# POSTECH-CVLab/PyTorch-StudioGAN

Hardware: AMD Instinct MI355X
Metric: images/sec (G+D step) BigGAN ImageNet-128 bs256 (higher is better)
Workload: dtype bf16

## Files before the change

pytorch-studiogan_amd/csrc/attn.hip:

```cpp
#include "common.h"
#include "lds_tile.h"
#include "../../include/sgamd.h"

#ifndef AT_UNROLL
#define AT_UNROLL 1
#endif
#ifndef AT_WAVES
#define AT_WAVES(NCG) ((NCG) <= 2 ? 3 : 2)
#endif

__device__ __forceinline__ u32x4 at_gfrag(const bf16_t* base, long long row, int ld, int c, int C) {
  u32x4 z = {0u, 0u, 0u, 0u};
  return (c < C) ? *(const u32x4*)(base + row * ld + c) : z;
}

#ifndef AT_THR
#define AT_THR 8.0f
#endif
template <int NCG>
__global__ __launch_bounds__(256) __attribute__((amdgpu_waves_per_eu(AT_WAVES(NCG), AT_WAVES(NCG)))) void k_attn_fwd_flash(const bf16_t* theta, const bf16_t* phi, const bf16_t* g, float* lse, bf16_t* O, float* O32,
                                                        int HW, int HW4, int Dp, int Cg) {
  constexpr int KC = 256;
  constexpr float LOG2E = 1.4426950408889634f;
  extern __shared__ __attribute__((aligned(16))) char at_smem[];
  char* kimg = at_smem;
  char* vimg = at_smem + KC * 64;
  const int tid = threadIdx.x, lane = tid & 63, wave = __builtin_amdgcn_readfirstlane(tid >> 6);
  const int b = blockIdx.y;
  const int q = blockIdx.x * 128 + wave * 32 + (lane & 31);
  const int h = lane >> 5;
  const long long qrow = (long long)b * HW + q;
  const bf16x8_t qf0 = __builtin_bit_cast(bf16x8_t, at_gfrag(theta, qrow, Dp, 8 * h, Dp));
  const bf16x8_t qf1 = __builtin_bit_cast(bf16x8_t, at_gfrag(theta, qrow, Dp, 16 + 8 * h, Dp));
  float m = -3.0e38f;
  float m2 = m * LOG2E;
  float l = 0.f;
  f32x16 o[NCG];
#pragma unroll
  for (int cg = 0; cg < NCG; cg++)
#pragma unroll
    for (int r = 0; r < 16; r++) o[cg][r] = 0.f;
  for (int k0 = 0; k0 < HW4; k0 += KC) {
    __syncthreads();
    lt_stage_cols<4>(kimg, phi + ((long long)b * HW4 + k0) * Dp, KC, Dp, 0, Dp, wave, lane);
#pragma unroll
    for (int cg = 0; cg < NCG; cg++) lt_stage_cols<4>(vimg + cg * KC * 64, g + ((long long)b * HW4 + k0) * Cg, KC, Cg, cg * 32, Cg, wave, lane);
    __syncthreads();
#pragma unroll AT_UNROLL
    for (int kc = 0; kc < KC / 32; kc++) {
      f32x16 s;
#pragma unroll
      for (int r = 0; r < 16; r++) s[r] = 0.f;
      s = __builtin_amdgcn_mfma_f32_32x32x16_bf16(lt_frag(kimg, kc, 0, lane), qf0, s, 0, 0, 0);
      s = __builtin_amdgcn_mfma_f32_32x32x16_bf16(lt_frag(kimg, kc, 1, lane), qf1, s, 0, 0, 0);
      float bm = s[0];
#pragma unroll
      for (int r = 1; r < 16; r++) bm = fmaxf(bm, s[r]);
      bm = lt_half_max(bm);
      if (bm > m + AT_THR) {
        const float alpha = __builtin_amdgcn_exp2f((m - bm) * LOG2E);
        l *= alpha;
#pragma unroll
        for (int cg = 0; cg < NCG; cg++)
#pragma unroll
          for (int r = 0; r < 16; r++) o[cg][r] *= alpha;
        m = bm;
        m2 = m * LOG2E;
      }
      float p[16];
#pragma unroll
      for (int r = 0; r < 16; r++) { p[r] = __builtin_amdgcn_exp2f(__builtin_fmaf(s[r], LOG2E, -m2)); l += p[r]; }
      u32x4 pa, pb;
#pragma unroll
      for (int i = 0; i < 4; i++) { pa[i] = pack2bf(p[2 * i], p[2 * i + 1]); pb[i] = pack2bf(p[8 + 2 * i], p[8 + 2 * i + 1]); }
      const bf16x8_t pfa = __builtin_bit_cast(bf16x8_t, pa), pfb = __builtin_bit_cast(bf16x8_t, pb);
#pragma unroll
      for (int cg = 0; cg < NCG; cg++) {
        const char* vi = vimg + cg * KC * 64;
        o[cg] = __builtin_amdgcn_mfma_f32_32x32x16_bf16(lt_vfrag(vi, kc * 32 + 4 * h, lane), pfa, o[cg], 0, 0, 0);
        o[cg] = __builtin_amdgcn_mfma_f32_32x32x16_bf16(lt_vfrag(vi, kc * 32 + 16 + 4 * h, lane), pfb, o[cg], 0, 0, 0);
      }
    }
  }
  l = lt_half_sum(l);
  const float inv = 1.f / l;
  if (h == 0) lse[qrow] = m + __logf(l);
  bf16_t* orow = O + qrow * Cg;
#pragma unroll
  for (int cg = 0; cg < NCG; cg++)
#pragma unroll
    for (int g4 = 0; g4 < 4; g4++) {
      const int c0 = cg * 32 + 8 * g4 + 4 * h;
      if (c0 < Cg) {
        const f32x4 f = {o[cg][4 * g4 + 0] * inv, o[cg][4 * g4 + 1] * inv, o[cg][4 * g4 + 2] * inv, o[cg][4 * g4 + 3] * inv};
        u32x2 v = {pack2bf(f[0], f[1]), pack2bf(f[2], f[3])};
        *(u32x2*)(orow + c0) = v;
        if (O32) *(f32x4*)(O32 + qrow * Cg + c0) = f;
      }
    }
}

template <int NCG> __global__ __launch_bounds__(256) __attribute__((amdgpu_waves_per_eu(AT_WAVES(NCG), AT_WAVES(NCG)))) void k_attn_bwd_q(const bf16_t* theta, const bf16_t* phi, const bf16_t* g, const bf16_t* dO, const float* Oin,
                                                                        const float* lse, float* delta_out, bf16_t* dtheta, int HW, int HW4, int Dp, int Cg) {
  constexpr int KC = 256;
  extern __shared__ __attribute__((aligned(16))) char at_smem[];
  char* kimg = at_smem;
  char* vimg = at_smem + KC * 64;
  const int tid = threadIdx.x, lane = tid & 63, wave = __builtin_amdgcn_readfirstlane(tid >> 6);
  const int b = blockIdx.y;
  const int q = blockIdx.x * 128 + wave * 32 + (lane & 31);
  const int h = lane >> 5;
  const long long qrow = (long long)b * HW + q;
  const bf16x8_t qf0 = __builtin_bit_cast(bf16x8_t, at_gfrag(theta, qrow, Dp, 8 * h, Dp));
  const bf16x8_t qf1 = __builtin_bit_cast(bf16x8_t, at_gfrag(theta, qrow, Dp, 16 + 8 * h, Dp));
  bf16x8_t df[NCG][2];
#pragma unroll
  for (int cg = 0; cg < NCG; cg++)
#pragma unroll
    for (int t = 0; t < 2; t++) df[cg][t] = __builtin_bit_cast(bf16x8_t, at_gfrag(dO, qrow, Cg, cg * 32 + 16 * t + 8 * h, Cg));
  float delta = 0.f;
  const float ls2 = lse[qrow] * 1.4426950408889634f;
  if (Oin) {
#pragma unroll
    for (int cg = 0; cg < NCG; cg++)
#pragma unroll
      for (int t = 0; t < 2; t++) {
        const int c0 = cg * 32 + 16 * t + 8 * h;
        if (c0 < Cg) {
          const f32x4 oa = *(const f32x4*)(Oin + qrow * Cg + c0), ob = *(const f32x4*)(Oin + qrow * Cg + c0 + 4);
          const u32x4 dv = __builtin_bit_cast(u32x4, df[cg][t]);
          delta += oa[0] * __uint_as_float(dv[0] << 16) + oa[1] * __uint_as_float(dv[0] & 0xffff0000u) + oa[2] * __uint_as_float(dv[1] << 16) + oa[3] * __uint_as_float(dv[1] & 0xffff0000u)
                 + ob[0] * __uint_as_float(dv[2] << 16) + ob[1] * __uint_as_float(dv[2] & 0xffff0000u) + ob[2] * __uint_as_float(dv[3] << 16) + ob[3] * __uint_as_float(dv[3] & 0xffff0000u);
        }
      }
    delta = lt_half_sum(delta);
  }
  f32x16 dth;
#pragma unroll
  for (int r = 0; r < 16; r++) dth[r] = 0.f;
  for (int pass = Oin ? 1 : 0; pass < 2; pass++) {
    for (int k0 = 0; k0 < HW4; k0 += KC) {
      __syncthreads();
      lt_stage_cols<4>(kimg, phi + ((long long)b * HW4 + k0) * Dp, KC, Dp, 0, Dp, wave, lane);
#pragma unroll
      for (int cg = 0; cg < NCG; cg++) lt_stage_cols<4>(vimg + cg * KC * 64, g + ((long long)b * HW4 + k0) * Cg, KC, Cg, cg * 32, Cg, wave, lane);
      __syncthreads();
#pragma unroll AT_UNROLL
      for (int kb = 0; kb < KC / 32; kb++) {
        f32x16 s, dp;
#pragma unroll
        for (int r = 0; r < 16; r++) { s[r] = 0.f; dp[r] = 0.f; }
        s = __builtin_amdgcn_mfma_f32_32x32x16_bf16(lt_frag(kimg, kb, 0, lane), qf0, s, 0, 0, 0);
        s = __builtin_amdgcn_mfma_f32_32x32x16_bf16(lt_frag(kimg, kb, 1, lane), qf1, s, 0, 0, 0);
#pragma unroll
        for (int cg = 0; cg < NCG; cg++)
#pragma unroll
          for (int t = 0; t < 2; t++)
            dp = __builtin_amdgcn_mfma_f32_32x32x16_bf16(lt_frag(vimg + cg * KC * 64, kb, t, lane), df[cg][t], dp, 0, 0, 0);
        if (pass == 0) {
#pragma unroll
          for (int r = 0; r < 16; r++) delta += __builtin_amdgcn_exp2f(__builtin_fmaf(s[r], 1.4426950408889634f, -ls2)) * dp[r];
        } else {
          float o[16];
#pragma unroll
          for (int r = 0; r < 16; r++) o[r] = __builtin_amdgcn_exp2f(__builtin_fmaf(s[r], 1.4426950408889634f, -ls2)) * (dp[r] - delta);
          u32x4 da, db;
#pragma unroll
          for (int i = 0; i < 4; i++) { da[i] = pack2bf(o[2 * i], o[2 * i + 1]); db[i] = pack2bf(o[8 + 2 * i], o[8 + 2 * i + 1]); }
          dth = __builtin_amdgcn_mfma_f32_32x32x16_bf16(lt_vfrag(kimg, kb * 32 + 4 * h, lane), __builtin_bit_cast(bf16x8_t, da), dth, 0, 0, 0);
          dth = __builtin_amdgcn_mfma_f32_32x32x16_bf16(lt_vfrag(kimg, kb * 32 + 16 + 4 * h, lane), __builtin_bit_cast(bf16x8_t, db), dth, 0, 0, 0);
        }
      }
    }
    if (pass == 0) delta = lt_half_sum(delta);
  }
  if (h == 0) delta_out[qrow] = delta;
  bf16_t* trow = dtheta + qrow * Dp;
#pragma unroll
  for (int g4 = 0; g4 < 4; g4++) {
    const int c0 = 8 * g4 + 4 * h;
    if (c0 < Dp) {
      u32x2 v = {pack2bf(dth[4 * g4 + 0], dth[4 * g4 + 1]), pack2bf(dth[4 * g4 + 2], dth[4 * g4 + 3])};
      *(u32x2*)(trow + c0) = v;
    }
  }
}

template <int NCG> __global__ __launch_bounds__(256) __attribute__((amdgpu_waves_per_eu(AT_WAVES(NCG), AT_WAVES(NCG)))) void k_attn_bwd_k(const bf16_t* theta, const bf16_t* phi, const bf16_t* g, const bf16_t* dO, const float* lse,
                                                                        const float* delta, bf16_t* dphi, bf16_t* dg, int HW, int HW4, int Dp, int Cg) {
  constexpr int QC = 256;
  extern __shared__ __attribute__((aligned(16))) char at_smem[];
  char* timg = at_smem;
  char* oimg = at_smem + QC * 64;
  float* st = (float*)(at_smem + (1 + NCG) * QC * 64);
  float* dl = st + QC;
  const int tid = threadIdx.x, lane = tid & 63, wave = __builtin_amdgcn_readfirstlane(tid >> 6);
  const int b = blockIdx.y;
  const int key = blockIdx.x * 128 + wave * 32 + (lane & 31);
  const int h = lane >> 5;
  const long long krow = (long long)b * HW4 + key;
  const bf16x8_t kf0 = __builtin_bit_cast(bf16x8_t, at_gfrag(phi, krow, Dp, 8 * h, Dp));
  const bf16x8_t kf1 = __builtin_bit_cast(bf16x8_t, at_gfrag(phi, krow, Dp, 16 + 8 * h, Dp));
  bf16x8_t gf[NCG][2];
#pragma unroll
  for (int cg = 0; cg < NCG; cg++)
#pragma unroll
    for (int t = 0; t < 2; t++) gf[cg][t] = __builtin_bit_cast(bf16x8_t, at_gfrag(g, krow, Cg, cg * 32 + 16 * t + 8 * h, Cg));
  f32x16 dph, dgt[NCG];
#pragma unroll
  for (int r = 0; r < 16; r++) dph[r] = 0.f;
#pragma unroll
  for (int cg = 0; cg < NCG; cg++)
#pragma unroll
    for (int r = 0; r < 16; r++) dgt[cg][r] = 0.f;
  for (int q0 = 0; q0 < HW; q0 += QC) {
    __syncthreads();
    lt_stage_cols<4>(timg, theta + ((long long)b * HW + q0) * Dp, QC, Dp, 0, Dp, wave, lane);
#pragma unroll
    for (int cg = 0; cg < NCG; cg++) lt_stage_cols<4>(oimg + cg * QC * 64, dO + ((long long)b * HW + q0) * Cg, QC, Cg, cg * 32, Cg, wave, lane);
    if (tid < QC) { st[tid] = lse[(long long)b * HW + q0 + tid] * 1.4426950408889634f; dl[tid] = delta[(long long)b * HW + q0 + tid]; }
    __syncthreads();
#pragma unroll AT_UNROLL
    for (int qb = 0; qb < QC / 32; qb++) {
      f32x16 s, dp;
#pragma unroll
      for (int r = 0; r < 16; r++) { s[r] = 0.f; dp[r] = 0.f; }
      s = __builtin_amdgcn_mfma_f32_32x32x16_bf16(lt_frag(timg, qb, 0, lane), kf0, s, 0, 0, 0);
      s = __builtin_amdgcn_mfma_f32_32x32x16_bf16(lt_frag(timg, qb, 1, lane), kf1, s, 0, 0, 0);
#pragma unroll
      for (int cg = 0; cg < NCG; cg++)
#pragma unroll
        for (int t = 0; t < 2; t++)
          dp = __builtin_amdgcn_mfma_f32_32x32x16_bf16(lt_frag(oimg + cg * QC * 64, qb, t, lane), gf[cg][t], dp, 0, 0, 0);
      float pr[16], ds[16];
#pragma unroll
      for (int r = 0; r < 16; r++) {
        const int qi = qb * 32 + (r & 3) + 8 * (r >> 2) + 4 * h;
        pr[r] = __builtin_amdgcn_exp2f(__builtin_fmaf(s[r], 1.4426950408889634f, -st[qi]));
        ds[r] = pr[r] * (dp[r] - dl[qi]);
      }
      u32x4 pa, pb, da, db;
#pragma unroll
      for (int i = 0; i < 4; i++) {
        pa[i] = pack2bf(pr[2 * i], pr[2 * i + 1]); pb[i] = pack2bf(pr[8 + 2 * i], pr[8 + 2 * i + 1]);
        da[i] = pack2bf(ds[2 * i], ds[2 * i + 1]); db[i] = pack2bf(ds[8 + 2 * i], ds[8 + 2 * i + 1]);
      }
#pragma unroll
      for (int cg = 0; cg < NCG; cg++) {
        const char* oi = oimg + cg * QC * 64;
        dgt[cg] = __builtin_amdgcn_mfma_f32_32x32x16_bf16(lt_vfrag(oi, qb * 32 + 4 * h, lane), __builtin_bit_cast(bf16x8_t, pa), dgt[cg], 0, 0, 0);
        dgt[cg] = __builtin_amdgcn_mfma_f32_32x32x16_bf16(lt_vfrag(oi, qb * 32 + 16 + 4 * h, lane), __builtin_bit_cast(bf16x8_t, pb), dgt[cg], 0, 0, 0);
      }
      dph = __builtin_amdgcn_mfma_f32_32x32x16_bf16(lt_vfrag(timg, qb * 32 + 4 * h, lane), __builtin_bit_cast(bf16x8_t, da), dph, 0, 0, 0);
      dph = __builtin_amdgcn_mfma_f32_32x32x16_bf16(lt_vfrag(timg, qb * 32 + 16 + 4 * h, lane), __builtin_bit_cast(bf16x8_t, db), dph, 0, 0, 0);
    }
  }
  bf16_t* prow = dphi + krow * Dp;
  bf16_t* grow = dg + krow * Cg;
#pragma unroll
  for (int g4 = 0; g4 < 4; g4++) {
    const int c0 = 8 * g4 + 4 * h;
    if (c0 < Dp) {
      u32x2 v = {pack2bf(dph[4 * g4 + 0], dph[4 * g4 + 1]), pack2bf(dph[4 * g4 + 2], dph[4 * g4 + 3])};
      *(u32x2*)(prow + c0) = v;
    }
  }
#pragma unroll
  for (int cg = 0; cg < NCG; cg++)
#pragma unroll
    for (int g4 = 0; g4 < 4; g4++) {
      const int c0 = cg * 32 + 8 * g4 + 4 * h;
      if (c0 < Cg) {
        u32x2 v = {pack2bf(dgt[cg][4 * g4 + 0], dgt[cg][4 * g4 + 1]), pack2bf(dgt[cg][4 * g4 + 2], dgt[cg][4 * g4 + 3])};
        *(u32x2*)(grow + c0) = v;
      }
    }
}

static bool at_ok(int B, int HW, int HW4, int Dp) {
  return B > 0 && B <= 65535 && HW % 128 == 0 && HW4 % 256 == 0 && Dp % 8 == 0 && Dp >= 8 && Dp <= 32;
}
extern "C" int sg_attn_fwd_flash_ok(int B, int HW, int HW4, int Dp, int Cg) {
  return (at_ok(B, HW, HW4, Dp) && Cg % 8 == 0 && Cg >= 8 && Cg <= 128) ? 1 : 0;
}
extern "C" int sg_attn_fwd_fused(const void* theta, const void* phi, const void* g, float* lse, void* O, float* O32, int B, int HW, int HW4, int Dp, int Cg, sg_stream_t s) {
  SG_CHECK(theta && phi && g && lse && O, "sg_attn_fwd_fused: null");
  SG_CHECK(sg_attn_fwd_flash_ok(B, HW, HW4, Dp, Cg) == 1, "sg_attn_fwd_fused: unsupported shape");
  const int ncg = (Cg + 31) / 32;
  SgProfScope prof((hipStream_t)s, (double)B * HW * ((Dp + Cg) * 2.0 + 4.0) + (double)B * HW4 * (Dp + Cg) * 2.0, 5);
  const dim3 grid(HW / 128, B), blk(256);
  hipStream_t st = (hipStream_t)s;
#define ATL_LAUNCH(N)                                                                                                                     \
  {                                                                                                                                        \
    static const bool ok = lt_allow_lds(k_attn_fwd_flash<N>, (1 + N) * 16384);                                                             \
    SG_CHECK(ok, "sg_attn_fwd_fused: LDS attribute");                                                                                      \
    hipLaunchKernelGGL((k_attn_fwd_flash<N>), grid, blk, (1 + N) * 16384, st, (const bf16_t*)theta, (const bf16_t*)phi, (const bf16_t*)g, lse, (bf16_t*)O, O32, HW, HW4, Dp, Cg); \
  }
  if (ncg == 1) ATL_LAUNCH(1) else if (ncg == 2) ATL_LAUNCH(2) else if (ncg == 3) ATL_LAUNCH(3) else ATL_LAUNCH(4)
#undef ATL_LAUNCH
  SG_LAUNCH_CHECK();
  return 0;
}
extern "C" int sg_attn_bwd_fused_ok(int B, int HW, int HW4, int Dp, int Cg) {
  return (at_ok(B, HW, HW4, Dp) && HW % 256 == 0 && HW4 % 128 == 0 && Cg % 8 == 0 && Cg >= 8 && Cg <= 128) ? 1 : 0;
}
extern "C" int sg_attn_bwd_fused(const void* theta, const void* phi, const void* g, const void* dO, const float* O32, const float* lse, float* delta, void* dtheta, void* dphi,
                                 void* dg, int B, int HW, int HW4, int Dp, int Cg, sg_stream_t s) {
  SG_CHECK(theta && phi && g && dO && lse && delta && dtheta && dphi && dg, "sg_attn_bwd_fused: null");
  SG_CHECK(sg_attn_bwd_fused_ok(B, HW, HW4, Dp, Cg) == 1, "sg_attn_bwd_fused: unsupported shape");
  const int ncg = (Cg + 31) / 32;
  const int lds_q = (1 + ncg) * 256 * 64, lds_k = (1 + ncg) * 256 * 64 + 2 * 256 * 4;
  SgProfScope prof((hipStream_t)s, 2.0 * ((double)B * HW * ((Dp + Cg) * 2.0 + 8.0) + (double)B * HW4 * (Dp + Cg) * 2.0) + (double)B * (HW + HW4) * (Dp * 2.0) + (double)B * HW4 * Cg * 2.0, 5);
  hipStream_t st = (hipStream_t)s;
#define ATB_LAUNCH(N)                                                                                                                     \
  {                                                                                                                                        \
    static const bool ok = lt_allow_lds(k_attn_bwd_q<N>, lds_q) && lt_allow_lds(k_attn_bwd_k<N>, lds_k);                                   \
    SG_CHECK(ok, "sg_attn_bwd_fused: LDS attribute");                                                                                      \
    hipLaunchKernelGGL(k_attn_bwd_q<N>, dim3(HW / 128, B), dim3(256), lds_q, st, (const bf16_t*)theta, (const bf16_t*)phi, (const bf16_t*)g, (const bf16_t*)dO, O32, lse, delta, (bf16_t*)dtheta, HW, HW4, Dp, Cg); \
    hipLaunchKernelGGL(k_attn_bwd_k<N>, dim3(HW4 / 128, B), dim3(256), lds_k, st, (const bf16_t*)theta, (const bf16_t*)phi, (const bf16_t*)g, (const bf16_t*)dO, lse, (const float*)delta, (bf16_t*)dphi, (bf16_t*)dg, HW, HW4, Dp, Cg); \
  }
  if (ncg == 1) ATB_LAUNCH(1) else if (ncg == 2) ATB_LAUNCH(2) else if (ncg == 3) ATB_LAUNCH(3) else ATB_LAUNCH(4)
#undef ATB_LAUNCH
  SG_LAUNCH_CHECK();
  return 0;
}
```

Baseline: 2065.

## Specialize attention kernels on head-dim and channel tail; use 128-key chunks

Adds template parameters so the attention forward and backward kernels skip the second QK MFMA when the projection dim fits in one 16-wide step. They also skip the last dP MFMA when the final 32-channel group has only 16 valid channels. The forward and query-backward kernels gain a 128-row staging chunk for wider channel counts, which halves LDS per block and allows higher waves-per-EU targets. This trades more template instantiations and an env-driven dispatch for fewer wasted zero-padded MFMAs and better occupancy, at the cost of more barrier/stage iterations per key sweep.

```diff
diff --git a/pytorch-studiogan_amd/csrc/attn.hip b/pytorch-studiogan_amd/csrc/attn.hip
--- a/pytorch-studiogan_amd/csrc/attn.hip
+++ b/pytorch-studiogan_amd/csrc/attn.hip
@@ -6,8 +6,12 @@
 #define AT_UNROLL 1
 #endif
 #ifndef AT_WAVES
-#define AT_WAVES(NCG) ((NCG) <= 2 ? 3 : 2)
+#define AT_WAVES(NCG, KC) ((KC) == 256 ? ((NCG) <= 2 ? 3 : 2) : ((NCG) <= 2 ? 4 : 3))
 #endif
+#ifndef AT_WAVES_FWD
+#define AT_WAVES_FWD(NCG, KC) ((KC) == 128 && (NCG) == 3 ? 4 : AT_WAVES(NCG, KC))
+#endif
+#define AT_DP_STEP(cg, t) ((cg) < NCG - 1 || (t) < NGL)
 
 __device__ __forceinline__ u32x4 at_gfrag(const bf16_t* base, long long row, int ld, int c, int C) {
   u32x4 z = {0u, 0u, 0u, 0u};
@@ -17,10 +21,9 @@
 #ifndef AT_THR
 #define AT_THR 8.0f
 #endif
-template <int NCG>
-__global__ __launch_bounds__(256) __attribute__((amdgpu_waves_per_eu(AT_WAVES(NCG), AT_WAVES(NCG)))) void k_attn_fwd_flash(const bf16_t* theta, const bf16_t* phi, const bf16_t* g, float* lse, bf16_t* O, float* O32,
+template <int NCG, int ND, int KC>
+__global__ __launch_bounds__(256) __attribute__((amdgpu_waves_per_eu(AT_WAVES_FWD(NCG, KC), AT_WAVES_FWD(NCG, KC)))) void k_attn_fwd_flash(const bf16_t* theta, const bf16_t* phi, const bf16_t* g, float* lse, bf16_t* O, float* O32,
                                                         int HW, int HW4, int Dp, int Cg) {
-  constexpr int KC = 256;
   constexpr float LOG2E = 1.4426950408889634f;
   extern __shared__ __attribute__((aligned(16))) char at_smem[];
   char* kimg = at_smem;
@@ -31,7 +34,7 @@
   const int h = lane >> 5;
   const long long qrow = (long long)b * HW + q;
   const bf16x8_t qf0 = __builtin_bit_cast(bf16x8_t, at_gfrag(theta, qrow, Dp, 8 * h, Dp));
-  const bf16x8_t qf1 = __builtin_bit_cast(bf16x8_t, at_gfrag(theta, qrow, Dp, 16 + 8 * h, Dp));
+  const bf16x8_t qf1 = __builtin_bit_cast(bf16x8_t, at_gfrag(theta, qrow, Dp, 16 + 8 * h, ND == 2 ? Dp : 0));
   float m = -3.0e38f;
   float m2 = m * LOG2E;
   float l = 0.f;
@@ -52,7 +55,7 @@
 #pragma unroll
       for (int r = 0; r < 16; r++) s[r] = 0.f;
       s = __builtin_amdgcn_mfma_f32_32x32x16_bf16(lt_frag(kimg, kc, 0, lane), qf0, s, 0, 0, 0);
-      s = __builtin_amdgcn_mfma_f32_32x32x16_bf16(lt_frag(kimg, kc, 1, lane), qf1, s, 0, 0, 0);
+      if constexpr (ND == 2) s = __builtin_amdgcn_mfma_f32_32x32x16_bf16(lt_frag(kimg, kc, 1, lane), qf1, s, 0, 0, 0);
       float bm = s[0];
 #pragma unroll
       for (int r = 1; r < 16; r++) bm = fmaxf(bm, s[r]);
@@ -100,9 +103,8 @@
     }
 }
 
-template <int NCG> __global__ __launch_bounds__(256) __attribute__((amdgpu_waves_per_eu(AT_WAVES(NCG), AT_WAVES(NCG)))) void k_attn_bwd_q(const bf16_t* theta, const bf16_t* phi, const bf16_t* g, const bf16_t* dO, const float* Oin,
+template <int NCG, int ND, int NGL, int KC> __global__ __launch_bounds__(256) __attribute__((amdgpu_waves_per_eu(AT_WAVES(NCG, KC), AT_WAVES(NCG, KC)))) void k_attn_bwd_q(const bf16_t* theta, const bf16_t* phi, const bf16_t* g, const bf16_t* dO, const float* Oin,
                                                                         const float* lse, float* delta_out, bf16_t* dtheta, int HW, int HW4, int Dp, int Cg) {
-  constexpr int KC = 256;
   extern __shared__ __attribute__((aligned(16))) char at_smem[];
   char* kimg = at_smem;
   char* vimg = at_smem + KC * 64;
@@ -112,12 +114,13 @@
   const int h = lane >> 5;
   const long long qrow = (long long)b * HW + q;
   const bf16x8_t qf0 = __builtin_bit_cast(bf16x8_t, at_gfrag(theta, qrow, Dp, 8 * h, Dp));
-  const bf16x8_t qf1 = __builtin_bit_cast(bf16x8_t, at_gfrag(theta, qrow, Dp, 16 + 8 * h, Dp));
+  const bf16x8_t qf1 = __builtin_bit_cast(bf16x8_t, at_gfrag(theta, qrow, Dp, 16 + 8 * h, ND == 2 ? Dp : 0));
   bf16x8_t df[NCG][2];
 #pragma unroll
   for (int cg = 0; cg < NCG; cg++)
 #pragma unroll
-    for (int t = 0; t < 2; t++) df[cg][t] = __builtin_bit_cast(bf16x8_t, at_gfrag(dO, qrow, Cg, cg * 32 + 16 * t + 8 * h, Cg));
+    for (int t = 0; t < 2; t++)
+      if (AT_DP_STEP(cg, t)) df[cg][t] = __builtin_bit_cast(bf16x8_t, at_gfrag(dO, qrow, Cg, cg * 32 + 16 * t + 8 * h, Cg));
   float delta = 0.f;
   const float ls2 = lse[qrow] * 1.4426950408889634f;
   if (Oin) {
@@ -126,7 +129,7 @@
 #pragma unroll
       for (int t = 0; t < 2; t++) {
         const int c0 = cg * 32 + 16 * t + 8 * h;
-        if (c0 < Cg) {
+        if (AT_DP_STEP(cg, t) && c0 < Cg) {
           const f32x4 oa = *(const f32x4*)(Oin + qrow * Cg + c0), ob = *(const f32x4*)(Oin + qrow * Cg + c0 + 4);
           const u32x4 dv = __builtin_bit_cast(u32x4, df[cg][t]);
           delta += oa[0] * __uint_as_float(dv[0] << 16) + oa[1] * __uint_as_float(dv[0] & 0xffff0000u) + oa[2] * __uint_as_float(dv[1] << 16) + oa[3] * __uint_as_float(dv[1] & 0xffff0000u)
@@ -151,12 +154,12 @@
 #pragma unroll
         for (int r = 0; r < 16; r++) { s[r] = 0.f; dp[r] = 0.f; }
         s = __builtin_amdgcn_mfma_f32_32x32x16_bf16(lt_frag(kimg, kb, 0, lane), qf0, s, 0, 0, 0);
-        s = __builtin_amdgcn_mfma_f32_32x32x16_bf16(lt_frag(kimg, kb, 1, lane), qf1, s, 0, 0, 0);
+        if constexpr (ND == 2) s = __builtin_amdgcn_mfma_f32_32x32x16_bf16(lt_frag(kimg, kb, 1, lane), qf1, s, 0, 0, 0);
 #pragma unroll
         for (int cg = 0; cg < NCG; cg++)
 #pragma unroll
           for (int t = 0; t < 2; t++)
-            dp = __builtin_amdgcn_mfma_f32_32x32x16_bf16(lt_frag(vimg + cg * KC * 64, kb, t, lane), df[cg][t], dp, 0, 0, 0);
+            if (AT_DP_STEP(cg, t)) dp = __builtin_amdgcn_mfma_f32_32x32x16_bf16(lt_frag(vimg + cg * KC * 64, kb, t, lane), df[cg][t], dp, 0, 0, 0);
         if (pass == 0) {
 #pragma unroll
           for (int r = 0; r < 16; r++) delta += __builtin_amdgcn_exp2f(__builtin_fmaf(s[r], 1.4426950408889634f, -ls2)) * dp[r];
@@ -186,9 +189,8 @@
   }
 }
 
-template <int NCG> __global__ __launch_bounds__(256) __attribute__((amdgpu_waves_per_eu(AT_WAVES(NCG), AT_WAVES(NCG)))) void k_attn_bwd_k(const bf16_t* theta, const bf16_t* phi, const bf16_t* g, const bf16_t* dO, const float* lse,
+template <int NCG, int ND, int NGL, int QC> __global__ __launch_bounds__(256) __attribute__((amdgpu_waves_per_eu(AT_WAVES(NCG, QC), AT_WAVES(NCG, QC)))) void k_attn_bwd_k(const bf16_t* theta, const bf16_t* phi, const bf16_t* g, const bf16_t* dO, const float* lse,
                                                                         const float* delta, bf16_t* dphi, bf16_t* dg, int HW, int HW4, int Dp, int Cg) {
-  constexpr int QC = 256;
   extern __shared__ __attribute__((aligned(16))) char at_smem[];
   char* timg = at_smem;
   char* oimg = at_smem + QC * 64;
@@ -200,12 +202,13 @@
   const int h = lane >> 5;
   const long long krow = (long long)b * HW4 + key;
   const bf16x8_t kf0 = __builtin_bit_cast(bf16x8_t, at_gfrag(phi, krow, Dp, 8 * h, Dp));
-  const bf16x8_t kf1 = __builtin_bit_cast(bf16x8_t, at_gfrag(phi, krow, Dp, 16 + 8 * h, Dp));
+  const bf16x8_t kf1 = __builtin_bit_cast(bf16x8_t, at_gfrag(phi, krow, Dp, 16 + 8 * h, ND == 2 ? Dp : 0));
   bf16x8_t gf[NCG][2];
 #pragma unroll
   for (int cg = 0; cg < NCG; cg++)
 #pragma unroll
-    for (int t = 0; t < 2; t++) gf[cg][t] = __builtin_bit_cast(bf16x8_t, at_gfrag(g, krow, Cg, cg * 32 + 16 * t + 8 * h, Cg));
+    for (int t = 0; t < 2; t++)
+      if (AT_DP_STEP(cg, t)) gf[cg][t] = __builtin_bit_cast(bf16x8_t, at_gfrag(g, krow, Cg, cg * 32 + 16 * t + 8 * h, Cg));
   f32x16 dph, dgt[NCG];
 #pragma unroll
   for (int r = 0; r < 16; r++) dph[r] = 0.f;
@@ -226,12 +229,12 @@
 #pragma unroll
       for (int r = 0; r < 16; r++) { s[r] = 0.f; dp[r] = 0.f; }
       s = __builtin_amdgcn_mfma_f32_32x32x16_bf16(lt_frag(timg, qb, 0, lane), kf0, s, 0, 0, 0);
-      s = __builtin_amdgcn_mfma_f32_32x32x16_bf16(lt_frag(timg, qb, 1, lane), kf1, s, 0, 0, 0);
+      if constexpr (ND == 2) s = __builtin_amdgcn_mfma_f32_32x32x16_bf16(lt_frag(timg, qb, 1, lane), kf1, s, 0, 0, 0);
 #pragma unroll
       for (int cg = 0; cg < NCG; cg++)
 #pragma unroll
         for (int t = 0; t < 2; t++)
-          dp = __builtin_amdgcn_mfma_f32_32x32x16_bf16(lt_frag(oimg + cg * QC * 64, qb, t, lane), gf[cg][t], dp, 0, 0, 0);
+          if (AT_DP_STEP(cg, t)) dp = __builtin_amdgcn_mfma_f32_32x32x16_bf16(lt_frag(oimg + cg * QC * 64, qb, t, lane), gf[cg][t], dp, 0, 0, 0);
       float pr[16], ds[16];
 #pragma unroll
       for (int r = 0; r < 16; r++) {
@@ -280,6 +283,19 @@
 static bool at_ok(int B, int HW, int HW4, int Dp) {
   return B > 0 && B <= 65535 && HW % 128 == 0 && HW4 % 256 == 0 && Dp % 8 == 0 && Dp >= 8 && Dp <= 32;
 }
+static bool at_ksteps_full() {
+  const char* e = getenv("SG_ATTN_KSTEPS");
+  return e && e[0] == 'f';
+}
+enum { AT_K_FWD, AT_K_BWD_Q };
+#define AT_FWD_128(C) C(2, 1, 128) C(2, 2, 128) C(3, 1, 128) C(3, 2, 128) C(4, 1, 128) C(4, 2, 128)
+#define AT_BWD_Q_128(C) C(3, 1, 1, 128) C(3, 1, 2, 128) C(3, 2, 1, 128) C(3, 2, 2, 128) C(4, 1, 1, 128) C(4, 1, 2, 128) C(4, 2, 1, 128) C(4, 2, 2, 128)
+static int at_chunk(int kernel, int ncg) {
+  const bool has128 = kernel == AT_K_FWD ? ncg >= 2 : ncg >= 3;
+  const char* e = getenv("SG_ATTN_KC");
+  return (has128 && !(e && atoi(e) == 256)) ? 128 : 256;
+}
+static constexpr int at_key(int ncg, int nd, int ngl, int kc) { return ((ncg * 4 + nd) * 4 + ngl) * 2 + (kc == 128 ? 1 : 0); }
 extern "C" int sg_attn_fwd_flash_ok(int B, int HW, int HW4, int Dp, int Cg) {
   return (at_ok(B, HW, HW4, Dp) && Cg % 8 == 0 && Cg >= 8 && Cg <= 128) ? 1 : 0;
 }
@@ -287,17 +303,23 @@
   SG_CHECK(theta && phi && g && lse && O, "sg_attn_fwd_fused: null");
   SG_CHECK(sg_attn_fwd_flash_ok(B, HW, HW4, Dp, Cg) == 1, "sg_attn_fwd_fused: unsupported shape");
   const int ncg = (Cg + 31) / 32;
+  const int nd = at_ksteps_full() ? 2 : (Dp + 15) / 16;
+  const int kc = at_chunk(AT_K_FWD, ncg);
   SgProfScope prof((hipStream_t)s, (double)B * HW * ((Dp + Cg) * 2.0 + 4.0) + (double)B * HW4 * (Dp + Cg) * 2.0, 5);
   const dim3 grid(HW / 128, B), blk(256);
   hipStream_t st = (hipStream_t)s;
-#define ATL_LAUNCH(N)                                                                                                                     \
-  {                                                                                                                                        \
-    static const bool ok = lt_allow_lds(k_attn_fwd_flash<N>, (1 + N) * 16384);                                                             \
+#define ATL_CASE(N, D, K)                                                                                                                  \
+  case at_key(N, D, 2, K): {                                                                                                               \
+    static const bool ok = lt_allow_lds(k_attn_fwd_flash<N, D, K>, (1 + N) * K * 64);                                                      \
     SG_CHECK(ok, "sg_attn_fwd_fused: LDS attribute");                                                                                      \
-    hipLaunchKernelGGL((k_attn_fwd_flash<N>), grid, blk, (1 + N) * 16384, st, (const bf16_t*)theta, (const bf16_t*)phi, (const bf16_t*)g, lse, (bf16_t*)O, O32, HW, HW4, Dp, Cg); \
-  }
-  if (ncg == 1) ATL_LAUNCH(1) else if (ncg == 2) ATL_LAUNCH(2) else if (ncg == 3) ATL_LAUNCH(3) else ATL_LAUNCH(4)
-#undef ATL_LAUNCH
+    hipLaunchKernelGGL((k_attn_fwd_flash<N, D, K>), grid, blk, (1 + N) * K * 64, st, (const bf16_t*)theta, (const bf16_t*)phi, (const bf16_t*)g, lse, (bf16_t*)O, O32, HW, HW4, Dp, Cg); \
+  } break;
+  switch (at_key(ncg, nd, 2, kc)) {
+    ATL_CASE(1, 1, 256) ATL_CASE(1, 2, 256) ATL_CASE(2, 1, 256) ATL_CASE(2, 2, 256) ATL_CASE(3, 1, 256) ATL_CASE(3, 2, 256) ATL_CASE(4, 1, 256) ATL_CASE(4, 2, 256)
+    AT_FWD_128(ATL_CASE)
+    default: SG_CHECK(false, "sg_attn_fwd_fused: no instantiation");
+  }
+#undef ATL_CASE
   SG_LAUNCH_CHECK();
   return 0;
 }
@@ -309,18 +331,39 @@
   SG_CHECK(theta && phi && g && dO && lse && delta && dtheta && dphi && dg, "sg_attn_bwd_fused: null");
   SG_CHECK(sg_attn_bwd_fused_ok(B, HW, HW4, Dp, Cg) == 1, "sg_attn_bwd_fused: unsupported shape");
   const int ncg = (Cg + 31) / 32;
-  const int lds_q = (1 + ncg) * 256 * 64, lds_k = (1 + ncg) * 256 * 64 + 2 * 256 * 4;
+  const bool full = at_ksteps_full();
+  const int nd = full ? 2 : (Dp + 15) / 16, ngl = full ? 2 : (Cg - 32 * (ncg - 1) + 15) / 16;
+  const int nd_k = (ncg == 2 && nd == 1 && ngl == 2) ? 2 : nd;
+  const int kc_q = at_chunk(AT_K_BWD_Q, ncg);
   SgProfScope prof((hipStream_t)s, 2.0 * ((double)B * HW * ((Dp + Cg) * 2.0 + 8.0) + (double)B * HW4 * (Dp + Cg) * 2.0) + (double)B * (HW + HW4) * (Dp * 2.0) + (double)B * HW4 * Cg * 2.0, 5);
   hipStream_t st = (hipStream_t)s;
-#define ATB_LAUNCH(N)                                                                                                                     \
-  {                                                                                                                                        \
-    static const bool ok = lt_allow_lds(k_attn_bwd_q<N>, lds_q) && lt_allow_lds(k_attn_bwd_k<N>, lds_k);                                   \
+#define ATQ_CASE(N, D, G, K)                                                                                                               \
+  case at_key(N, D, G, K): {                                                                                                               \
+    static const bool ok = lt_allow_lds(k_attn_bwd_q<N, D, G, K>, (1 + N) * K * 64);                                                       \
     SG_CHECK(ok, "sg_attn_bwd_fused: LDS attribute");                                                                                      \
-    hipLaunchKernelGGL(k_attn_bwd_q<N>, dim3(HW / 128, B), dim3(256), lds_q, st, (const bf16_t*)theta, (const bf16_t*)phi, (const bf16_t*)g, (const bf16_t*)dO, O32, lse, delta, (bf16_t*)dtheta, HW, HW4, Dp, Cg); \
-    hipLaunchKernelGGL(k_attn_bwd_k<N>, dim3(HW4 / 128, B), dim3(256), lds_k, st, (const bf16_t*)theta, (const bf16_t*)phi, (const bf16_t*)g, (const bf16_t*)dO, lse, (const float*)delta, (bf16_t*)dphi, (bf16_t*)dg, HW, HW4, Dp, Cg); \
-  }
-  if (ncg == 1) ATB_LAUNCH(1) else if (ncg == 2) ATB_LAUNCH(2) else if (ncg == 3) ATB_LAUNCH(3) else ATB_LAUNCH(4)
-#undef ATB_LAUNCH
+    hipLaunchKernelGGL((k_attn_bwd_q<N, D, G, K>), dim3(HW / 128, B), dim3(256), (1 + N) * K * 64, st, (const bf16_t*)theta, (const bf16_t*)phi, (const bf16_t*)g, (const bf16_t*)dO, O32, lse, delta, (bf16_t*)dtheta, HW, HW4, Dp, Cg); \
+  } break;
+#define ATK_CASE(N, D, G, K)                                                                                                               \
+  case at_key(N, D, G, K): {                                                                                                               \
+    static const bool ok = lt_allow_lds(k_attn_bwd_k<N, D, G, K>, (1 + N) * K * 64 + 2 * K * 4);                                           \
+    SG_CHECK(ok, "sg_attn_bwd_fused: LDS attribute");                                                                                      \
+    hipLaunchKernelGGL((k_attn_bwd_k<N, D, G, K>), dim3(HW4 / 128, B), dim3(256), (1 + N) * K * 64 + 2 * K * 4, st, (const bf16_t*)theta, (const bf16_t*)phi, (const bf16_t*)g, (const bf16_t*)dO, lse, (const float*)delta, (bf16_t*)dphi, (bf16_t*)dg, HW, HW4, Dp, Cg); \
+  } break;
+#define AT_ALL_256(C, N) C(N, 1, 1, 256) C(N, 1, 2, 256) C(N, 2, 1, 256) C(N, 2, 2, 256)
+#define AT_K2_256(C) C(2, 1, 1, 256) C(2, 2, 1, 256) C(2, 2, 2, 256)
+  switch (at_key(ncg, nd, ngl, kc_q)) {
+    AT_ALL_256(ATQ_CASE, 1) AT_ALL_256(ATQ_CASE, 2) AT_ALL_256(ATQ_CASE, 3) AT_ALL_256(ATQ_CASE, 4)
+    AT_BWD_Q_128(ATQ_CASE)
+    default: SG_CHECK(false, "sg_attn_bwd_fused: no instantiation (query side)");
+  }
+  switch (at_key(ncg, nd_k, ngl, 256)) {
+    AT_ALL_256(ATK_CASE, 1) AT_K2_256(ATK_CASE) AT_ALL_256(ATK_CASE, 3) AT_ALL_256(ATK_CASE, 4)
+    default: SG_CHECK(false, "sg_attn_bwd_fused: no instantiation (key side)");
+  }
+#undef AT_K2_256
+#undef AT_ALL_256
+#undef ATK_CASE
+#undef ATQ_CASE
   SG_LAUNCH_CHECK();
   return 0;
 }
```

After: 2075 (median of 6 runs). Within noise of the previous version (+0.5%).
